# chanchanchan97/ICAFusion

Measured on NVIDIA H100. Metric: 640x512 RGB+IR pairs/sec end-to-end, higher is better.
Workload: dtype f16

## Files before the change

icafusion_b200/csrc/conv_common.cuh:

```cuda
#pragma once
#include "icaf_internal.cuh"

namespace icaf {

constexpr int BM = 128;
constexpr int BK = 64;
constexpr int kLag = 2;
constexpr int kThreads = 288;

enum AMode { A_GATHER = 0, A_TMA2D = 1, A_TMA4D = 2 };

struct ConvProblem {
  const __half* x; const float* bias; const __half* res; __half* y;
  const float* alpha; const float* beta;
  long long x_ld, res_ld, y_ld;
  const float2* ln_stats;
  const float* ln_s;
  float2* stats_out;
};
struct ConvParams {
  ConvProblem p[2];
  int M, N, K, k_pad;
  int B, Hi, Wi, Cin, Ho, Wo, kh, kw, stride, pad;
  int act, epi;
// ... 23 lines not shown
  r.y_ld = z ? P.p[1].y_ld : P.p[0].y_ld;
  r.ln_stats = z ? P.p[1].ln_stats : P.p[0].ln_stats; r.ln_s = z ? P.p[1].ln_s : P.p[0].ln_s;
  r.stats_out = z ? P.p[1].stats_out : P.p[0].stats_out;
  return r;
}

struct TileOrigin { int m0, tb, oy0, ox0; };
__device__ __forceinline__ void tile_origin(const ConvParams& P, int mtile, int& m0, int& tb, int& oy0, int& ox0) {
  m0 = mtile * BM; tb = 0; oy0 = 0; ox0 = 0;
  if (P.a_mode == A_TMA4D) {
    const int per_img = P.tiles_x * P.tiles_y;
    m0 = 0;
    tb = mtile / per_img;
    const int t = mtile - tb * per_img;
    oy0 = (t / P.tiles_x) * P.th;
    ox0 = (t % P.tiles_x) * P.tw;
  }
}

__device__ __forceinline__ void tile_row(const ConvParams& P, const TileOrigin& o, int row, int& m, bool& valid) {
  if (P.a_mode == A_TMA4D) {
    const int ry = row / P.tw, rx = row - ry * P.tw;
    m = (o.tb * P.Ho + o.oy0 + ry) * P.Wo + o.ox0 + rx;
    valid = ry < P.th && o.oy0 + ry < P.Ho;
  } else {
    m = o.m0 + row;
    valid = m < P.M;
  }
}

struct EpiRow {
  float ln_a, ln_mu;
  const float* ln_s;
  float sum, sumsq;
};
__device__ __forceinline__ void epi_row_ln(EpiRow& ex, const ConvParams& P, const ConvProblem& pr, int m, bool mvalid) {
  float su = 0.f, sq = 0.f;
  if (mvalid) {
    const float2* sp = pr.ln_stats + size_t(m) * P.ln_parts;
    for (int i = 0; i < P.ln_parts; ++i) { const float2 v = __ldg(sp + i); su += v.x; sq += v.y; }
  }
  const float mu = su * P.ln_inv_k;
  ex.ln_mu = mu;
  ex.ln_a = rsqrtf(fmaxf(sq * P.ln_inv_k - mu * mu, 0.f) + P.ln_eps);
}

struct StagedRow {
  int m;
  bool mvalid;
  float rbias;
  __half* yrow;
  const __half* rrow;
  EpiRow ex;
};
template <int BN, bool XM>
__device__ __forceinline__ void staged_row(StagedRow& r, const ConvParams& P, const ConvProblem& pr, const TileOrigin& o, int row, int n0) {
  tile_row(P, o, row, r.m, r.mvalid);
  r.rbias = ((P.epi & ICAF_EPI_BIAS_ROW) && pr.bias && r.mvalid) ? __ldg(pr.bias + r.m) : 0.f;
  r.yrow = pr.y + size_t(r.mvalid ? r.m : 0) * pr.y_ld;
  r.rrow = pr.res ? pr.res + size_t(r.mvalid ? r.m : 0) * pr.res_ld : nullptr;
  if (r.rrow && r.mvalid) {
    for (int cb = 0; cb < BN && n0 + cb < P.N; cb += 64) prefetch_l2(r.rrow + n0 + cb);
  }
  r.ex.sum = r.ex.sumsq = 0.f; r.ex.ln_a = 1.f; r.ex.ln_mu = 0.f; r.ex.ln_s = nullptr;
  if (XM) {
    r.ex.ln_s = pr.ln_s ? pr.ln_s + n0 : nullptr;
    if (P.ln_parts > 0) epi_row_ln(r.ex, P, pr, r.m, r.mvalid);
  }
}

__device__ __forceinline__ void epi_row_emit(const EpiRow& ex, const ConvParams& P, const ConvProblem& pr, int m, int n_begin, int n_end) {
  const int slots = (P.N + 31) >> 5;
  float2* sp = pr.stats_out + size_t(m) * slots;
  const int s0 = n_begin >> 5, s1 = min((n_end + 31) >> 5, slots);
  for (int i = s0; i < s1; ++i) sp[i] = i == s0 ? make_float2(ex.sum, ex.sumsq) : make_float2(0.f, 0.f);
}

template <int ACT, int RES>
__device__ __forceinline__ float epi_value(float a, float b, float rbias, float rf, float alpha, float beta) {
  float t = a + b + rbias;
  if (ACT == ICAF_ACT_SILU) t = silu_f(t);
  if (ACT == ICAF_ACT_GELU) t = gelu_erf_f(t);
  if (RES == 1) t = t + rf;
  if (RES == 2) t = alpha * rf + beta * t;
  return t;
}

template <int ACT, int RES, int XM = 0>
__device__ __forceinline__ void epi_chunk(const uint32_t (&acc)[32], const float* __restrict__ sb, float rbias,
                                          float alpha, float beta, const __half* __restrict__ rp,
                                          __half* __restrict__ yp, bool vec, int ncols, EpiRow& ex, int cb, bool do_store = true) {
  auto f = [&](int j, float rf) {
    float a = __uint_as_float(acc[j]);
    if (XM == 1) a = ex.ln_a * (a - ex.ln_mu * __ldg(ex.ln_s + cb + j));
    return epi_value<ACT, RES>(a, sb[j], rbias, rf, alpha, beta);
  };
  if (vec) {
#pragma unroll
    for (int q = 0; q < 4; ++q) {
      float rf[8];
      if (RES != 0) {
        uint4 rr = *reinterpret_cast<const uint4*>(rp + q * 8);
        const __half2* rh = reinterpret_cast<const __half2*>(&rr);
#pragma unroll
        for (int e = 0; e < 4; ++e) {
          const float2 r2 = __half22float2(rh[e]);
          rf[2 * e] = r2.x; rf[2 * e + 1] = r2.y;
        }
      } else {
#pragma unroll
        for (int e = 0; e < 8; ++e) rf[e] = 0.f;
      }
      float v[8];
#pragma unroll
      for (int e = 0; e < 8; ++e) v[e] = f(q * 8 + e, rf[e]);
      uint4 o;
      o.x = pack_half2(v[0], v[1]); o.y = pack_half2(v[2], v[3]);
      o.z = pack_half2(v[4], v[5]); o.w = pack_half2(v[6], v[7]);
      if (XM == 2) {
        const __half2* oh = reinterpret_cast<const __half2*>(&o);
#pragma unroll
        for (int e = 0; e < 4; ++e) {
          const float2 w = __half22float2(oh[e]);
          ex.sum += w.x + w.y;
          ex.sumsq += w.x * w.x + w.y * w.y;
        }
      }
      if (do_store) *reinterpret_cast<uint4*>(yp + q * 8) = o;
    }
  } else {
#pragma unroll
    for (int j = 0; j < 32; ++j) {
      if (j < ncols) {
        const float t = f(j, RES != 0 ? __half2float(rp[j]) : 0.f);
        const __half h = __float2half_rn(t);
        if (XM == 2) { const float w = __half2float(h); ex.sum += w; ex.sumsq += w * w; }
        yp[j] = h;
      }
    }
  }
}

__device__ __forceinline__ void load_staged(uint32_t (&acc)[32], const float* p) {
#pragma unroll
  for (int q = 0; q < 8; ++q) {
    const float4 v = *reinterpret_cast<const float4*>(p + 4 * q);
    acc[4 * q] = __float_as_uint(v.x); acc[4 * q + 1] = __float_as_uint(v.y);
    acc[4 * q + 2] = __float_as_uint(v.z); acc[4 * q + 3] = __float_as_uint(v.w);
  }
}

template <bool XM>
__device__ __forceinline__ void epi_dispatch(int mode_act, const uint32_t (&acc)[32], const float* sb, float rbias, float alpha,
                                             float beta, const __half* rp, __half* yp, bool vec, int ncols, EpiRow& ex, int cb) {
  if (XM) {
    switch (mode_act) {
      case 9: epi_chunk<0, 0, 1>(acc, sb, rbias, alpha, beta, rp, yp, vec, ncols, ex, cb); break;
      case 10: epi_chunk<2, 0, 1>(acc, sb, rbias, alpha, beta, rp, yp, vec, ncols, ex, cb); break;
      default: epi_chunk<0, 2, 2>(acc, sb, rbias, alpha, beta, rp, yp, vec, ncols, ex, cb); break;
    }
  } else {
    switch (mode_act) {
      case 0: epi_chunk<0, 0>(acc, sb, rbias, alpha, beta, rp, yp, vec, ncols, ex, cb); break;
      case 1: epi_chunk<0, 1>(acc, sb, rbias, alpha, beta, rp, yp, vec, ncols, ex, cb); break;
      case 2: epi_chunk<0, 2>(acc, sb, rbias, alpha, beta, rp, yp, vec, ncols, ex, cb); break;
      case 3: epi_chunk<1, 0>(acc, sb, rbias, alpha, beta, rp, yp, vec, ncols, ex, cb); break;
      case 4: epi_chunk<1, 1>(acc, sb, rbias, alpha, beta, rp, yp, vec, ncols, ex, cb); break;
      case 5: epi_chunk<1, 2>(acc, sb, rbias, alpha, beta, rp, yp, vec, ncols, ex, cb); break;
      case 6: epi_chunk<2, 0>(acc, sb, rbias, alpha, beta, rp, yp, vec, ncols, ex, cb); break;
      case 7: epi_chunk<2, 1>(acc, sb, rbias, alpha, beta, rp, yp, vec, ncols, ex, cb); break;
      default: epi_chunk<2, 2>(acc, sb, rbias, alpha, beta, rp, yp, vec, ncols, ex, cb); break;
    }
  }
}

template <bool XM>
__device__ __forceinline__ int epi_mode_act(const ConvParams& P, bool has_res) {
  if (XM) return P.ln_parts > 0 ? (P.act == ICAF_ACT_GELU ? 10 : 9) : 11;
  return P.act * 3 + ((P.epi & ICAF_EPI_SCALED_RES) ? 2 : (has_res ? 1 : 0));
}

template <bool XM>
__device__ __forceinline__ void epi_staged_chunk(int mode_act, const uint32_t (&acc)[32], StagedRow& r, const float* sbias,
                                                 float alpha, float beta, int cb, int nb, int N) {
  const int ncols = min(32, N - nb);
  const bool vec = ncols == 32 && ((reinterpret_cast<uintptr_t>(r.yrow + nb) & 15) == 0) &&
                   (!r.rrow || (reinterpret_cast<uintptr_t>(r.rrow + nb) & 15) == 0);
  epi_dispatch<XM>(mode_act, acc, sbias + cb, r.rbias, alpha, beta, r.rrow ? r.rrow + nb : nullptr, r.yrow + nb, vec, ncols,
                   r.ex, cb);
}

constexpr int kOutHalfBytes = BM * 64 * 2;

template <int PP, int NA>
__device__ __forceinline__ void take_cols16(const float (&acc0)[NA], const float (&acc1)[NA], float (&v)[16]) {
  constexpr int Q = PP < NA / 8 ? PP : NA / 8 - 1;
#pragma unroll
  for (int e = 0; e < 8; ++e) { v[e] = acc0[8 * Q + e]; v[8 + e] = acc1[8 * Q + e]; }
}

template <int ACT, int RES>
__device__ __forceinline__ void epi_fragments(const float (&v)[16], uint32_t sa, const float* sb, const float (&rb)[4],
                                              float alpha, float beta) {
#pragma unroll
  for (int h = 0; h < 2; ++h) {
    uint32_t r[4];
    if (RES != 0) ldmatrix_x4(r, sa + 8192u * h);
#pragma unroll
    for (int k = 0; k < 4; ++k) {
      const float2 b = *reinterpret_cast<const float2*>(sb + 8 * (k >> 1));
      const float rbias = rb[2 * h + (k & 1)];
      float2 rf = make_float2(0.f, 0.f);
      if (RES != 0) rf = __half22float2(*reinterpret_cast<const __half2*>(&r[k]));
      r[k] = pack_half2(epi_value<ACT, RES>(v[8 * h + 2 * k], b.x, rbias, rf.x, alpha, beta),
                        epi_value<ACT, RES>(v[8 * h + 2 * k + 1], b.y, rbias, rf.y, alpha, beta));
    }
    stmatrix_x4(sa + 8192u * h, r);
  }
}

__device__ __forceinline__ void epi_fragments_dispatch(int mode_act, const float (&v)[16], uint32_t sa, const float* sb,
                                                       const float (&rb)[4], float alpha, float beta) {
  switch (mode_act) {
    case 0: epi_fragments<0, 0>(v, sa, sb, rb, alpha, beta); break;
    case 1: epi_fragments<0, 1>(v, sa, sb, rb, alpha, beta); break;
    case 2: epi_fragments<0, 2>(v, sa, sb, rb, alpha, beta); break;
    case 3: epi_fragments<1, 0>(v, sa, sb, rb, alpha, beta); break;
    case 4: epi_fragments<1, 1>(v, sa, sb, rb, alpha, beta); break;
    case 5: epi_fragments<1, 2>(v, sa, sb, rb, alpha, beta); break;
    case 6: epi_fragments<2, 0>(v, sa, sb, rb, alpha, beta); break;
    case 7: epi_fragments<2, 1>(v, sa, sb, rb, alpha, beta); break;
    default: epi_fragments<2, 2>(v, sa, sb, rb, alpha, beta); break;
  }
}

template <int NA>
__device__ __forceinline__ void epi_tile_fragments(int mode_act, const float (&acc0)[NA], const float (&acc1)[NA], uint32_t sout,
                                                   const float* sbias, const float (&rb)[4], float alpha, float beta, int w, int l) {
  const uint32_t sa = sout + uint32_t(16 * w + (l & 7) + 8 * ((l >> 3) & 1)) * 128u;
  const float* sb = sbias + 2 * (l & 3);
#pragma unroll 1
  for (int p = 0; p < NA / 8; ++p) {
    float v[16];
    switch (p) {
      case 0: take_cols16<0>(acc0, acc1, v); break;
      case 1: take_cols16<1>(acc0, acc1, v); break;
      case 2: take_cols16<2>(acc0, acc1, v); break;
      case 3: take_cols16<3>(acc0, acc1, v); break;
      case 4: take_cols16<4>(acc0, acc1, v); break;
      case 5: take_cols16<5>(acc0, acc1, v); break;
      case 6: take_cols16<6>(acc0, acc1, v); break;
      default: take_cols16<7>(acc0, acc1, v); break;
    }
    const uint32_t a = sa + uint32_t(p >> 2) * uint32_t(kOutHalfBytes) + (uint32_t((2 * (p & 3) + (l >> 4)) ^ (l & 7)) << 4);
    epi_fragments_dispatch(mode_act, v, a, sb + 16 * p, rb, alpha, beta);
  }
}

__device__ __forceinline__ void fragment_row_bias(float (&rb)[4], const ConvParams& P, const ConvProblem& pr, const TileOrigin& o,
                                                  int w, int l) {
  if ((P.epi & ICAF_EPI_BIAS_ROW) && pr.bias) {
#pragma unroll
    for (int q = 0; q < 4; ++q) {
      int mq;
      bool vq;
      tile_row(P, o, 16 * w + (l >> 2) + 8 * (q & 1) + 64 * (q >> 1), mq, vq);
      rb[q] = vq ? __ldg(pr.bias + mq) : 0.f;
    }
  }
}

template <int BN>
__device__ __forceinline__ void tma_store_tile(const ConvParams& P, const CUtensorMap* map, uint32_t s, int n0, const TileOrigin& o) {
  const int halves = (BN == 128 && n0 + 64 < P.N) ? 2 : 1;
  for (int hh = 0; hh < halves; ++hh) {
    const uint32_t src = s + uint32_t(hh * kOutHalfBytes);
    if (P.a_mode == A_TMA4D) tma_store_4d(map, src, n0 + 64 * hh, o.ox0, o.oy0, o.tb);
    else tma_store_2d(map, src, n0 + 64 * hh, o.m0);
  }
  bulk_commit_group();
}

template <int BN>
__device__ __forceinline__ void tma_load_tile(const ConvParams& P, const CUtensorMap* map, uint32_t s, uint32_t bar, int n0,
                                              const TileOrigin& o) {
  const int halves = (BN == 128 && n0 + 64 < P.N) ? 2 : 1;
  const uint32_t half_bytes = P.a_mode == A_TMA4D ? uint32_t(P.tw * P.th) * 128u : uint32_t(kOutHalfBytes);
  mbar_arrive_expect_tx(bar, uint32_t(halves) * half_bytes);
  for (int hh = 0; hh < halves; ++hh) {
    const uint32_t dst = s + uint32_t(hh * kOutHalfBytes);
    if (P.a_mode == A_TMA4D) tma_load_4d(dst, map, bar, n0 + 64 * hh, o.ox0, o.oy0, o.tb);
    else tma_load_2d(dst, map, bar, n0 + 64 * hh, o.m0);
  }
}

struct ConvPlan {
  int kernel;
  int bn;
  unsigned grid_x, grid_y, grid_z, cluster;
  int smem;
  int tiles, m_tiles, n_tiles;
  int sms;
  bool persist;
  bool xm;
  int ctas;
};

}
```

icafusion_b200/csrc/conv_gemm.cu:

```cuda
#include <cstdlib>
#include <cstring>

#include "conv_common.cuh"

namespace icaf {

constexpr int kMaxStages = 10;
template <int BN>
struct SmemLayout {
  static constexpr int kABytes = BM * BK * 2;
  static constexpr int kBBytes = BN * BK * 2;
  static constexpr int kStageBytes = kABytes + kBBytes;
  static constexpr int kPitch = BN + 4;
  static constexpr int kAccBytes = BM * kPitch * 4;
  static constexpr int kTailBytes = 256 + BN * 4 + 1024;
  __host__ __device__ static int region(int stages) { return stages * kStageBytes > kAccBytes ? stages * kStageBytes : kAccBytes; }
  static int total(int stages) { return region(stages) + kTailBytes; }
};


template <int BN, bool kTmaA>
__device__ __forceinline__ void load_stage(const ConvParams& P, int a_mode, uint32_t sa, uint32_t bar, uint32_t bytes,
                                           const CUtensorMap* mw, const CUtensorMap* ma, int kb, int n0, const TileOrigin& o) {
  mbar_arrive_expect_tx(bar, bytes);
// ... 229 lines not shown
      *reinterpret_cast<float2*>(sacc + size_t(r) * L::kPitch + col) = make_float2(acc0[i], acc0[i + 1]);
      *reinterpret_cast<float2*>(sacc + size_t(r + 64) * L::kPitch + col) = make_float2(acc1[i], acc1[i + 1]);
    }
    if (splits > 1) { cluster_arrive(); cluster_wait(); cluster_arrive(); cluster_wait(); } else { named_bar_sync(1, 256); }
  } else {
    if (elect_one()) {
      const CUtensorMap* mw = bz ? &maps.w[1] : &maps.w[0];
      const CUtensorMap* ma = bz ? &maps.a[1] : &maps.a[0];
      const uint32_t a_bytes = a_mode == A_TMA2D ? L::kABytes : (a_mode == A_TMA4D ? uint32_t(P.tw * P.th) * 128u : 0u);
      const uint32_t bytes = L::kBBytes + a_bytes;
      int s = 0;
      uint32_t ph = 0;
      for (int kb = 0; kb < nkb; ++kb) {
        mbar_wait_quiet(empty_bar(s), ph ^ 1);
        load_stage<BN, false>(P, a_mode, smem_base + s * L::kStageBytes, full_bar(s), bytes, mw, ma, kb_begin + kb, n0, o);
        if (++s == kStages) { s = 0; ph ^= 1; }
      }
      if (tma_epi && has_res) {
        mbar_wait_quiet(empty_bar(s), ph ^ 1);
        tma_load_tile<BN>(P, bz ? &maps.res[1] : &maps.res[0], smem_base + uint32_t(s) * L::kStageBytes, res_bar, n0, o);
      }
    }
    __syncwarp();
    if (splits > 1) { cluster_arrive(); cluster_wait(); cluster_arrive(); cluster_wait(); }
  }
}

constexpr int kPersistThreads = 384;
constexpr int kHaloSlots = 2;
struct PersistLayout {
  static constexpr int kStageBytes = SmemLayout<128>::kStageBytes;
  static constexpr int kFilterBytes = SmemLayout<128>::kBBytes;
  static constexpr int kOutBytes = 2 * kOutHalfBytes;
  static constexpr int kPitch = 32 + 4;
  static constexpr int kChunkBytes = BM * kPitch * 4;
  static_assert(kChunkBytes <= kOutBytes, "the XM staged chunk lives in the output tile");
  __host__ __device__ static int ring_bytes(int stages, int halo_bytes) {
    return halo_bytes ? stages * kFilterBytes + kHaloSlots * halo_bytes : stages * kStageBytes;
  }
  __host__ __device__ static int bar_off(int stages, int halo_bytes) { return ring_bytes(stages, halo_bytes) + 2 * kOutBytes; }
  static int total(int stages, int halo_bytes) { return bar_off(stages, halo_bytes) + 256 + 2 * 128 * 4 + 1024; }
};

template <class FullBar, class HaloFull, class HandBack, class HaloBack>
__device__ __forceinline__ void halo_mma_loop(float (&acc0)[64], float (&acc1)[64], const ConvParams& P, uint32_t smem_base,
                                              int kStages, int g0, int h0, const int (&lane_px)[2], int l, FullBar full_bar,
                                              HaloFull halo_full, HandBack hand_back, HaloBack halo_back, int& s_last, int& h_last) {
  const int ncb = P.Cin / BK, hw = P.tw + 2;
  const uint32_t halo_base = smem_base + uint32_t(kStages * PersistLayout::kFilterBytes);
  int s = g0 % kStages, h = h0 % kHaloSlots;
  uint32_t ph = uint32_t(g0 / kStages) & 1u, hph = uint32_t(h0 / kHaloSlots) & 1u;
  int s_prev = s, h_prev = h;
  uint32_t fa[3][4][4];
  for (int cb = 0; cb < ncb; ++cb) {
    mbar_wait_quiet(halo_full(h), hph);
    const uint32_t sh = halo_base + uint32_t(h * P.halo_bytes);
#pragma unroll 1
    for (int ky = 0; ky < 3; ++ky) {
#pragma unroll
      for (int kx = 0; kx < 3; ++kx) {
        const int tap = 3 * ky + kx;
        mbar_wait_quiet(full_bar(s), ph);
        const uint32_t sb = smem_base + uint32_t(s * PersistLayout::kFilterBytes);
#pragma unroll
        for (int hm = 0; hm < 2; ++hm) {
          const int f = (2 * kx + hm) % 3;
          const int r = lane_px[hm] + ky * hw + kx;
          const uint32_t a = sh + uint32_t(r) * 128u;
#pragma unroll
          for (int kc = 0; kc < 4; ++kc) ldmatrix_x4(fa[f][kc], a + (uint32_t((2 * kc + (l >> 4)) ^ (r & 7)) << 4));
          wgmma_fence();
#pragma unroll
          for (int kc = 0; kc < 4; ++kc) {
            const uint64_t bd = gmma_desc_sw128(sb + 32 * kc);
            if (hm == 0) wgmma_rs<0>(acc0, fa[f][kc], bd, (cb | tap | kc) != 0);
            else wgmma_rs<0>(acc1, fa[f][kc], bd, (cb | tap | kc) != 0);
          }
          wgmma_commit();
          wgmma_wait<2>();
          if (hm == 1 && (cb | tap) != 0) {
            hand_back(s_prev);
            if (tap == 0) halo_back(h_prev);
          }
        }
        s_prev = s;
        if (++s == kStages) { s = 0; ph ^= 1; }
      }
    }
    h_prev = h;
    if (++h == kHaloSlots) { h = 0; hph ^= 1; }
  }
  s_last = s_prev;
  h_last = h_prev;
}

struct PersistTile { int z, n0; TileOrigin o; };
__device__ __forceinline__ PersistTile persist_tile(const ConvParams& P, int t) {
  PersistTile pt;
  const int r = t / P.n_tiles;
  const int mtile = r % P.m_tiles;
  pt.n0 = (t - r * P.n_tiles) * 128;
  pt.z = r / P.m_tiles;
  tile_origin(P, mtile, pt.o.m0, pt.o.tb, pt.o.oy0, pt.o.ox0);
  return pt;
}

template <int CC>
__device__ __forceinline__ void stage_chunk(const float (&acc0)[64], const float (&acc1)[64], float* sacc, int w, int l) {
#pragma unroll
  for (int i = 16 * CC; i < 16 * CC + 16; i += 2) {
    const int r = 16 * w + (l >> 2) + 8 * ((i >> 1) & 1), col = 8 * (i >> 2) - 32 * CC + 2 * (l & 3);
    *reinterpret_cast<float2*>(sacc + r * PersistLayout::kPitch + col) = make_float2(acc0[i], acc0[i + 1]);
    *reinterpret_cast<float2*>(sacc + (r + 64) * PersistLayout::kPitch + col) = make_float2(acc1[i], acc1[i + 1]);
  }
}

template <bool XM>
__global__ void __launch_bounds__(kPersistThreads, 1)
conv_gemm_persist_kernel(const ConvParams P, const __grid_constant__ ConvMaps maps) {
  extern __shared__ uint8_t smem_raw[];
  const uint32_t smem_base = (smem_u32(smem_raw) + 1023u) & ~1023u;
  using L = SmemLayout<128>;
  using PL = PersistLayout;
  const int kStages = P.stages;
  const bool halo = !XM && P.halo_bytes != 0;
  const uint32_t ring_bytes = uint32_t(PL::ring_bytes(kStages, P.halo_bytes));
  const uint32_t bar_off = uint32_t(PL::bar_off(kStages, P.halo_bytes));
  const uint32_t bar_base = smem_base + bar_off;
  auto full_bar = [&](int s) { return bar_base + 8u * s; };
  auto empty_bar = [&](int s) { return bar_base + 8u * (kMaxStages + s); };
  auto order_bar = [&](int c) { return bar_base + 8u * (2 * kMaxStages + c); };
  auto res_bar = [&](int c) { return bar_base + 8u * (2 * kMaxStages + 2 + c); };
  auto halo_full = [&](int h) { return bar_base + 8u * (2 * kMaxStages + 4 + h); };
  auto halo_empty = [&](int h) { return bar_base + 8u * (2 * kMaxStages + 4 + kHaloSlots + h); };
  static_assert(8 * (2 * kMaxStages + 4 + 2 * kHaloSlots) <= 256, "barriers");
  uint8_t* smem_gen = smem_raw + (smem_base - smem_u32(smem_raw));

  pdl_launch_dependents();
  const int tid = threadIdx.x;
  const int wg = tid >> 7;
  const int ncb = P.Cin / BK;
  const int nkb = halo ? 9 * ncb : P.k_pad / BK;
  const int a_mode = P.a_mode;
  const bool has_res = (P.epi & (ICAF_EPI_ADD_RES | ICAF_EPI_SCALED_RES)) != 0;
  if (tid == 0) {
    for (int s = 0; s < kStages; ++s) {
      mbar_init(full_bar(s), 1);
      mbar_init(empty_bar(s), 4);
    }
    mbar_init(order_bar(0), 4);
    mbar_init(order_bar(1), 4);
    mbar_init(res_bar(0), 1);
    mbar_init(res_bar(1), 1);
    for (int h = 0; h < kHaloSlots; ++h) {
      mbar_init(halo_full(h), 1);
      mbar_init(halo_empty(h), 4);
    }
    fence_mbar_init();
  }
  if (tid == 32) {
    tma_prefetch_desc(&maps.w[0]);
    tma_prefetch_desc(&maps.a[0]);
    if (P.tiles > P.m_tiles * P.n_tiles) { tma_prefetch_desc(&maps.w[1]); tma_prefetch_desc(&maps.a[1]); }
    if (!XM) {
      tma_prefetch_desc(&maps.y[0]);
      if (has_res) tma_prefetch_desc(&maps.res[0]);
    }
  }
  __syncthreads();
  pdl_wait();

  if (wg == 0) {
    setmaxnreg_dec<40>();
    if (tid < 32 && elect_one()) {
      const uint32_t a_bytes = a_mode == A_TMA2D ? L::kABytes : uint32_t(P.tw * P.th) * 128u;
      const uint32_t bytes = L::kBBytes + a_bytes;
      int s = 0, h = 0;
      uint32_t ph = 0, hph = 0;
      for (int tile = blockIdx.x; tile < P.tiles; tile += gridDim.x) {
        const PersistTile pt = persist_tile(P, tile);
        const CUtensorMap* mw = pt.z ? &maps.w[1] : &maps.w[0];
        const CUtensorMap* ma = pt.z ? &maps.a[1] : &maps.a[0];
        if (halo) {
          const uint32_t halo_tx = uint32_t((P.tw + 2) * (P.th + 2)) * 128u;
          for (int cb = 0; cb < ncb; ++cb) {
            mbar_wait_quiet(halo_empty(h), hph ^ 1);
            mbar_arrive_expect_tx(halo_full(h), halo_tx);
            tma_load_4d(smem_base + uint32_t(kStages * PL::kFilterBytes + h * P.halo_bytes), ma, halo_full(h), cb * BK,
                        pt.o.ox0 - 1, pt.o.oy0 - 1, pt.o.tb);
            if (++h == kHaloSlots) { h = 0; hph ^= 1; }
            for (int tap = 0; tap < 9; ++tap) {
              mbar_wait_quiet(empty_bar(s), ph ^ 1);
              mbar_arrive_expect_tx(full_bar(s), PL::kFilterBytes);
              tma_load_2d(smem_base + uint32_t(s * PL::kFilterBytes), mw, full_bar(s), tap * P.Cin + cb * BK, pt.n0);
              if (++s == kStages) { s = 0; ph ^= 1; }
            }
          }
          continue;
        }
        for (int kb = 0; kb < nkb; ++kb) {
          mbar_wait_quiet(empty_bar(s), ph ^ 1);
          load_stage<128, true>(P, a_mode, smem_base + s * L::kStageBytes, full_bar(s), bytes, mw, ma, kb, pt.n0, pt.o);
          if (++s == kStages) { s = 0; ph ^= 1; }
        }
      }
    }
    return;
  }

  setmaxnreg_inc<232>();
  const int c = wg - 1;
  const int t = tid & 127, w = t >> 5, l = t & 31;
  const int bar_id = 2 + c;
  const uint32_t sout = smem_base + ring_bytes + uint32_t(c * PL::kOutBytes);
  float* sacc = reinterpret_cast<float*>(smem_gen + ring_bytes + c * PL::kOutBytes);
  float* sbias = reinterpret_cast<float*>(smem_gen + bar_off + 256 + c * 128 * 4);
  int lane_px[2];
#pragma unroll
  for (int hm = 0; hm < 2; ++hm) {
    int m = 64 * hm + 16 * w + (l & 7) + 8 * ((l >> 3) & 1);
    if (m > P.tw * P.th - 1) m = P.tw * P.th - 1;
    const int py = P.tw ? m / P.tw : 0;
    lane_px[hm] = py * (P.tw + 2) + m - py * P.tw;
  }
  for (int tile = blockIdx.x + c * gridDim.x; tile < P.tiles; tile += 2 * gridDim.x) {
    const int j = (tile - int(blockIdx.x)) / int(gridDim.x);
    const PersistTile pt = persist_tile(P, tile);
    const ConvProblem pr = pick_problem(P, pt.z);
    const int n0 = pt.n0;
    const TileOrigin& o = pt.o;
    const float bias_r = (pr.bias && !(P.epi & ICAF_EPI_BIAS_ROW) && n0 + t < P.N) ? __ldg(pr.bias + n0 + t) : 0.f;
    float alpha = 0.f, beta = 1.f;
    if (P.epi & ICAF_EPI_SCALED_RES) { alpha = __ldg(pr.alpha); beta = __ldg(pr.beta); }
    StagedRow sr;
    float rb[4] = {0.f, 0.f, 0.f, 0.f};
    if (XM) {
      staged_row<128, XM>(sr, P, pr, o, t, n0);
    } else {
      fragment_row_bias(rb, P, pr, o, w, l);
      if (t == 0) {
        bulk_wait_group_read<0>();
        if (has_res) tma_load_tile<128>(P, pt.z ? &maps.res[1] : &maps.res[0], sout, res_bar(c), n0, o);
      }
      sbias[t] = bias_r;
      named_bar_sync(bar_id, 128);
    }

    float acc0[64], acc1[64];
#pragma unroll
    for (int i = 0; i < 64; ++i) { acc0[i] = 0.f; acc1[i] = 0.f; }
    auto hand_back = [&](int s) { if (l == 0) mbar_arrive(empty_bar(s)); };
    auto halo_back = [&](int h) { if (l == 0) mbar_arrive(halo_empty(h)); };
    const int g0 = j * nkb;
    if (j > 0) mbar_wait_quiet(order_bar(c), uint32_t((j >> 1) - (1 - c)) & 1u);
    int s_last, h_last = 0;
    if (halo) {
      halo_mma_loop(acc0, acc1, P, smem_base, kStages, g0, j * ncb, lane_px, l, full_bar, halo_full, hand_back, halo_back,
                    s_last, h_last);
    } else {
      s_last = mma_loop<128>(acc0, acc1, smem_base, kStages, nkb, g0 % kStages, uint32_t(g0 / kStages) & 1u, full_bar,
                             hand_back);
    }
    if (l == 0) mbar_arrive(order_bar(c ^ 1));
    wgmma_wait<0>();
    hand_back(s_last);
    if (halo) halo_back(h_last);

    if constexpr (!XM) {
      if (has_res) mbar_wait_quiet(res_bar(c), uint32_t(j >> 1) & 1u);
      epi_tile_fragments<64>(epi_mode_act<false>(P, has_res), acc0, acc1, sout, sbias, rb, alpha, beta, w, l);
      fence_proxy_async_smem();
      named_bar_sync(bar_id, 128);
      if (t == 0) {
        tma_store_tile<128>(P, pt.z ? &maps.y[1] : &maps.y[0], sout, n0, o);
        if (tile + 2 * int(gridDim.x) >= P.tiles) bulk_wait_group<0>();
      }
      continue;
    }

    const int mode_act = epi_mode_act<XM>(P, has_res);
    const float* arow = sacc + size_t(t) * PL::kPitch;
#pragma unroll 1
    for (int cc = 0; cc < 4; ++cc) {
      named_bar_sync(bar_id, 128);
      if (cc == 0) sbias[t] = bias_r;
      switch (cc) {
        case 0: stage_chunk<0>(acc0, acc1, sacc, w, l); break;
        case 1: stage_chunk<1>(acc0, acc1, sacc, w, l); break;
        case 2: stage_chunk<2>(acc0, acc1, sacc, w, l); break;
        default: stage_chunk<3>(acc0, acc1, sacc, w, l); break;
      }
      named_bar_sync(bar_id, 128);
      const int cb = 32 * cc;
      if (sr.mvalid && n0 + cb < P.N) {
        uint32_t acc[32];
        load_staged(acc, arow);
        epi_staged_chunk<XM>(mode_act, acc, sr, sbias, alpha, beta, cb, n0 + cb, P.N);
      }
    }
    if (mode_act == 11 && sr.mvalid && n0 < P.N) epi_row_emit(sr.ex, P, pr, sr.m, n0, min(n0 + 128, P.N));
  }
}

struct SimtParams { ConvParams P; const __half* w[2]; };
__global__ void conv_gemm_simt_kernel(const SimtParams S) {
  pdl_launch_dependents();
  pdl_wait();
  const ConvParams& P = S.P;
  const ConvProblem pr = pick_problem(P, blockIdx.z);
  const __half* w = blockIdx.z ? S.w[1] : S.w[0];
  long long idx = blockIdx.x * (long long)blockDim.x + threadIdx.x;
  if (idx >= (long long)P.M * P.N) return;
  int n = int(idx % P.N);
  int m = int(idx / P.N);
  int ox = m % P.Wo, t = m / P.Wo, oy = t % P.Ho, b = t / P.Ho;
  float acc = 0.f;
  for (int ky = 0; ky < P.kh; ++ky)
    for (int kx = 0; kx < P.kw; ++kx) {
      int iy = oy * P.stride - P.pad + ky, ix = ox * P.stride - P.pad + kx;
      if ((unsigned)iy >= (unsigned)P.Hi || (unsigned)ix >= (unsigned)P.Wi) continue;
      const __half* xp = pr.x + (size_t(b) * P.Hi * P.Wi + size_t(iy) * P.Wi + ix) * pr.x_ld;
      const __half* wp = w + size_t(n) * P.k_pad + (ky * P.kw + kx) * P.Cin;
      for (int c = 0; c < P.Cin; ++c) acc += __half2float(xp[c]) * __half2float(wp[c]);
    }
  if (pr.bias) acc += (P.epi & ICAF_EPI_BIAS_ROW) ? pr.bias[m] : pr.bias[n];
  if (P.act == ICAF_ACT_SILU) acc = acc / (1.0f + expf(-acc));
  else if (P.act == ICAF_ACT_GELU) acc = gelu_erf_f(acc);
  if (pr.res) {
    float rf = __half2float(pr.res[size_t(m) * pr.res_ld + n]);
    acc = (P.epi & ICAF_EPI_SCALED_RES) ? (*pr.alpha) * rf + (*pr.beta) * acc : acc + rf;
  }
  pr.y[size_t(m) * pr.y_ld + n] = __float2half_rn(acc);
}

static int fill_geom(const icaf_conv_geom* g, int n_io, ConvParams& P) {
  if (!g || n_io < 1 || n_io > 2) return set_error(ICAF_ERR_BAD_ARG, "conv2d: need 1 or 2 problems");
  if (!(g->Cin == 4 || g->Cin % 8 == 0)) return set_error(ICAF_ERR_UNSUPPORTED, "conv2d: Cin must be 4 or a multiple of 8");
  if (g->Cin == 4 && (g->Wi % 2 || g->stride % 2 || g->pad % 2 || g->kw % 2))
    return set_error(ICAF_ERR_UNSUPPORTED, "conv2d: packed-image (Cin=4) path needs even Wi, stride, pad, kw");
  if (g->k_pad % 64 || g->k_pad < g->kh * g->kw * g->Cin) return set_error(ICAF_ERR_BAD_ARG, "conv2d: bad k_pad");
  if (g->w_rows < g->Cout) return set_error(ICAF_ERR_BAD_ARG, "conv2d: w_rows < Cout");
  long long M = (long long)g->B * g->Ho * g->Wo;
  if (M <= 0 || M > 0x7fffffffLL || (long long)g->B * g->Hi * g->Wi > 0x7fffffffLL)
    return set_error(ICAF_ERR_BAD_ARG, "conv2d: size out of range");
  if ((g->epi & (ICAF_EPI_ADD_RES | ICAF_EPI_SCALED_RES)) == (ICAF_EPI_ADD_RES | ICAF_EPI_SCALED_RES))
    return set_error(ICAF_ERR_BAD_ARG, "conv2d: ADD_RES and SCALED_RES are exclusive");
  if ((g->epi & ICAF_EPI_LN_FOLD) && ((g->epi & ~ICAF_EPI_LN_FOLD) != 0 || !(g->act == ICAF_ACT_NONE || g->act == ICAF_ACT_GELU) ||
                                      g->kh != 1 || g->kw != 1 || g->stride != 1 || g->pad != 0))
    return set_error(ICAF_ERR_UNSUPPORTED, "conv2d: LN_FOLD is a linear-layer (1x1) epilogue without residual, activation none / GELU");
  if ((g->epi & ICAF_EPI_EMIT_STATS) && ((g->epi & ~ICAF_EPI_EMIT_STATS) != ICAF_EPI_SCALED_RES || g->act != ICAF_ACT_NONE))
    return set_error(ICAF_ERR_UNSUPPORTED, "conv2d: EMIT_STATS rides on the SCALED_RES epilogue without activation");
  P.M = int(M); P.N = g->Cout; P.K = g->kh * g->kw * g->Cin; P.k_pad = g->k_pad;
  P.B = g->B; P.Hi = g->Hi; P.Wi = g->Wi; P.Cin = g->Cin; P.Ho = g->Ho; P.Wo = g->Wo;
  P.kh = g->kh; P.kw = g->kw; P.stride = g->stride; P.pad = g->pad; P.act = g->act; P.epi = g->epi;
  P.a_mode = A_GATHER; P.tw = P.th = P.tiles_x = P.tiles_y = 0; P.stages = 2; P.splits = 1; P.cblk = 64;
  P.ln_parts = 0; P.ln_eps = 0.f; P.ln_inv_k = 0.f;
  P.m_tiles = P.n_tiles = P.tiles = 0;
  P.tma_epi = 0;
  P.halo_bytes = 0;
  memset(P.p, 0, sizeof(P.p));
  return ICAF_OK;
}

static int fill_params(const icaf_conv_geom* g, const icaf_conv_io* io, int n_io, ConvParams& P, const __half* (&w)[2]) {
  if (!io) return set_error(ICAF_ERR_BAD_ARG, "conv2d: null io");
  if (int rc = fill_geom(g, n_io, P)) return rc;
  for (int i = 0; i < 2; ++i) {
    const icaf_conv_io& s = io[i < n_io ? i : 0];
    bool need_res = g->epi & (ICAF_EPI_ADD_RES | ICAF_EPI_SCALED_RES);
    if (!s.x || !s.w || !s.y || (need_res && !s.res) || ((g->epi & ICAF_EPI_SCALED_RES) && (!s.alpha || !s.beta)))
      return set_error(ICAF_ERR_BAD_ARG, "conv2d: null pointer");
    if ((reinterpret_cast<uintptr_t>(s.x) & 15) || (reinterpret_cast<uintptr_t>(s.w) & 15) || (s.x_ld % 8 && g->Cin != 4) ||
        (g->Cin == 4 && s.x_ld != 4))
      return set_error(ICAF_ERR_BAD_ARG, "conv2d: x / w must be 16-byte aligned with x_ld a multiple of 8");
    if ((g->epi & ICAF_EPI_LN_FOLD) && (!s.ln_stats || !s.ln_colsum || s.ln_parts < 1 || s.ln_parts > 64))
      return set_error(ICAF_ERR_BAD_ARG, "conv2d: LN_FOLD needs ln_stats, ln_colsum and 1..64 partials per row");
    if ((g->epi & ICAF_EPI_EMIT_STATS) && !s.stats_out) return set_error(ICAF_ERR_BAD_ARG, "conv2d: EMIT_STATS needs stats_out");
    if (i > 0 && (g->epi & ICAF_EPI_LN_FOLD) && (s.ln_parts != io[0].ln_parts || s.ln_eps != io[0].ln_eps))
      return set_error(ICAF_ERR_BAD_ARG, "conv2d: grouped problems must share ln_parts / ln_eps");
    P.p[i] = ConvProblem{(const __half*)s.x, s.bias, need_res ? (const __half*)s.res : nullptr, (__half*)s.y, s.alpha, s.beta,
                         s.x_ld, s.res_ld, s.y_ld,
                         (g->epi & ICAF_EPI_LN_FOLD) ? (const float2*)s.ln_stats : nullptr,
                         (g->epi & ICAF_EPI_LN_FOLD) ? s.ln_colsum : nullptr,
                         (g->epi & ICAF_EPI_EMIT_STATS) ? (float2*)s.stats_out : nullptr};
    if (i == 0 && (g->epi & ICAF_EPI_LN_FOLD)) { P.ln_parts = s.ln_parts; P.ln_eps = s.ln_eps; P.ln_inv_k = 1.0f / float(P.K); }
    w[i] = (const __half*)s.w;
  }
  return ICAF_OK;
}

static void plan_a_mode(const icaf_conv_geom* g, ConvParams& P) {
  if (g->kh == 1 && g->kw == 1 && g->stride == 1 && g->pad == 0 && g->Cin % 8 == 0) {
    P.a_mode = A_TMA2D;
    return;
  }
  if (g->Cin % 64 == 0 && g->stride <= 2) {
    int best_tw = 0, best_th = 0;
    double best_u = 0.0;
    for (int tw = 1; tw <= 128 && tw <= g->Wo; ++tw) {
      if (g->Wo % tw || tw * g->stride > 256) continue;
      int th = 128 / tw;
      if (th > g->Ho) th = g->Ho;
      if (th * g->stride > 256) th = 256 / g->stride;
      int ty = (g->Ho + th - 1) / th;
      double u = double(g->Wo) * g->Ho / (double(g->Wo / tw) * ty * 128.0);
      if (u > best_u + 1e-9 || (u > best_u - 1e-9 && tw > best_tw)) { best_u = u; best_tw = tw; best_th = th; }
    }
    if (best_u >= 0.6) {
      P.a_mode = A_TMA4D; P.tw = best_tw; P.th = best_th; P.tiles_x = g->Wo / best_tw; P.tiles_y = (g->Ho + best_th - 1) / best_th;
    }
  }
}

template <int BN>
static int plan_tc(ConvParams& P, int n_io, ConvPlan& pl) {
  using L = SmemLayout<BN>;
  constexpr int kSmemCap = 227 * 1024;
  const int mt = P.a_mode == A_TMA4D ? P.B * P.tiles_x * P.tiles_y : (P.M + BM - 1) / BM;
  if (P.a_mode == A_TMA4D && !(P.tw >= 1 && P.th >= 1 && P.tw * P.th <= BM && P.tiles_x * P.tw >= P.Wo && P.tiles_y * P.th >= P.Ho &&
                               P.cblk == 64 && P.Cin % 64 == 0))
    return set_error(ICAF_ERR_BAD_ARG, "conv2d(tc): 4-D tiles must cover the map with at most 128 pixels each, 64-channel blocks");
  unsigned gx = unsigned(mt), gy = unsigned((P.N + BN - 1) / BN), gz = unsigned(n_io);
  const long long tiles = (long long)gx * gy * gz;
  const int budget = (tiles <= pl.sms || BN > 64) ? kSmemCap : (kSmemCap / 2 - 1024);
  int stages = (budget - L::kTailBytes) / L::kStageBytes;
  const int nkb = P.k_pad / BK;
  if (stages > nkb) stages = nkb;
  if (stages > kMaxStages) stages = kMaxStages;
  if (stages < 2) stages = 2;
  int splits = 1;
  if (tiles * 2 <= pl.sms && nkb >= 8) {
    splits = int(pl.sms / tiles);
    if (splits > 8) splits = 8;
    if (splits > nkb / 4) splits = nkb / 4;
    if (splits < 1) splits = 1;
  }
  if (splits > 1) {
    const int per = (nkb + splits - 1) / splits;
    if (stages > per) stages = per < 2 ? 2 : per;
    gx *= splits;
  }
  if (stages > kMaxStages || L::total(stages) > kSmemCap)
    return set_error(ICAF_ERR_BAD_ARG, "conv2d(tc): shared-memory plan exceeds the ring / 227 KB");
  P.stages = stages;
  P.splits = splits;
  pl.kernel = ICAF_KERNEL_TC; pl.bn = BN;
  pl.grid_x = gx; pl.grid_y = gy; pl.grid_z = gz; pl.cluster = unsigned(splits);
  pl.smem = L::total(stages);
  pl.tiles = int(tiles); pl.m_tiles = mt; pl.n_tiles = int(gy);
  pl.persist = false; pl.ctas = int(gx * gy * gz);
  return ICAF_OK;
}

static int plan_persist(ConvParams& P, ConvPlan& pl) {
  constexpr int kSmemCap = 227 * 1024;
  const bool halo = !pl.xm && P.a_mode == A_TMA4D && P.kh == 3 && P.kw == 3 && P.stride == 1 && P.pad == 1;
  P.halo_bytes = halo ? ((P.tw + 2) * (P.th + 2) * 128 + 1023) / 1024 * 1024 : 0;
  int stages = kMaxStages;
  while (stages > 2 && PersistLayout::total(stages, P.halo_bytes) > kSmemCap) --stages;
  if (PersistLayout::total(stages, P.halo_bytes) > kSmemCap)
    return set_error(ICAF_ERR_BAD_ARG, "conv2d(persist): shared-memory plan exceeds 227 KB");
  P.stages = stages;
  P.m_tiles = pl.m_tiles; P.n_tiles = pl.n_tiles; P.tiles = pl.tiles;
  pl.persist = true;
  pl.ctas = pl.tiles < pl.sms ? pl.tiles : pl.sms;
  pl.smem = PersistLayout::total(stages, P.halo_bytes);
  return ICAF_OK;
}

template <int BN>
static int encode_maps(const ConvParams& P, const __half* const (&w)[2], const icaf_conv_geom* g, int n_io, bool out_maps,
                       ConvMaps& maps) {
  memset(&maps, 0, sizeof(maps));
  for (int i = 0; i < n_io; ++i) {
    int rc = encode_tmap_2d(&maps.w[i], w[i], (uint64_t)P.k_pad, (uint64_t)g->w_rows, (uint64_t)P.k_pad * 2, BK, BN);
    if (rc) return rc;
    const ConvProblem& pr = P.p[i];
    if (P.a_mode == A_TMA2D)
      rc = encode_tmap_2d(&maps.a[i], pr.x, (uint64_t)P.Cin, (uint64_t)P.M, (uint64_t)pr.x_ld * 2, BK, BM);
    else if (P.a_mode == A_TMA4D && P.halo_bytes)
      rc = encode_tmap_nhwc(&maps.a[i], pr.x, P.Cin, P.Wi, P.Hi, P.B, pr.x_ld, BK, P.tw + 2, P.th + 2, 1, 1);
    else if (P.a_mode == A_TMA4D)
      rc = encode_tmap_nhwc(&maps.a[i], pr.x, P.Cin, P.Wi, P.Hi, P.B, pr.x_ld, BK, P.tw * P.stride, P.th * P.stride, P.stride,
                            P.stride);
    if (rc) return rc;
    if (out_maps) {
      auto out_map = [&](CUtensorMap* m, const __half* base, long long ld) {
        return P.a_mode != A_TMA4D ? encode_tmap_2d(m, base, (uint64_t)P.N, (uint64_t)P.M, (uint64_t)ld * 2, 64, BM)
                                   : encode_tmap_nhwc(m, base, P.N, P.Wo, P.Ho, P.B, ld, 64, P.tw, P.th, 1, 1);
      };
      if ((rc = out_map(&maps.y[i], pr.y, pr.y_ld))) return rc;
      if (pr.res && (rc = out_map(&maps.res[i], pr.res, pr.res_ld))) return rc;
    }
  }
  if (n_io == 1) { maps.w[1] = maps.w[0]; maps.a[1] = maps.a[0]; maps.y[1] = maps.y[0]; maps.res[1] = maps.res[0]; }
  return ICAF_OK;
}

template <int BN>
static int launch_conv(const ConvParams& P, const ConvPlan& pl, const __half* const (&w)[2], const icaf_conv_geom* g, int n_io,
                       cudaStream_t st) {
  void (*kernel)(ConvParams, ConvMaps) = pl.xm ? conv_gemm_tc_kernel<BN, true> : conv_gemm_tc_kernel<BN, false>;
  if (pl.persist) kernel = pl.xm ? conv_gemm_persist_kernel<true> : conv_gemm_persist_kernel<false>;
  static bool configured[2][2][kMaxDevices] = {};
  if (int rc = configure_smem(kernel, 227 * 1024, configured[pl.persist][pl.xm], "conv2d: cudaFuncSetAttribute")) return rc;
  ConvMaps maps;
  if (int rc = encode_maps<BN>(P, w, g, n_io, P.tma_epi != 0, maps)) return rc;
  const dim3 grid = pl.persist ? dim3(unsigned(pl.ctas)) : dim3(pl.grid_x, pl.grid_y, pl.grid_z);
  return launch_kc("conv2d_fwd", kernel, grid, dim3(pl.persist ? kPersistThreads : kThreads), (size_t)pl.smem, st, pl.cluster, P, maps);
}

static int plan_conv(const icaf_conv_geom* g, int n_io, int sms, bool tma_out, ConvParams& P, ConvPlan& pl) {
  memset(&pl, 0, sizeof(pl));
  pl.sms = sms;
  if (sms < 1) return set_error(ICAF_ERR_BAD_ARG, "conv2d: SM count must be positive");
  pl.xm = (P.epi & (ICAF_EPI_LN_FOLD | ICAF_EPI_EMIT_STATS)) != 0;
  plan_a_mode(g, P);
  const long long mt = P.a_mode == A_TMA4D ? (long long)P.B * P.tiles_x * P.tiles_y : (P.M + BM - 1) / BM;
  auto ctas = [&](int bn) { return mt * ((P.N + bn - 1) / bn) * n_io; };
  int bn = 32;
  if (P.N > 64 && ctas(128) >= sms) bn = 128;
  else if (P.N > 32 && ctas(64) >= sms) bn = 64;
  int rc;
  switch (bn) {
    case 128:
      rc = plan_tc<128>(P, n_io, pl);
      if (!rc && (pl.xm || tma_out) && P.a_mode != A_GATHER && P.splits == 1 && pl.tiles > sms) rc = plan_persist(P, pl);
      break;
    case 64: rc = plan_tc<64>(P, n_io, pl); break;
    default: rc = plan_tc<32>(P, n_io, pl); break;
  }
  if (rc) return rc;
  P.tma_epi = !pl.xm && (pl.persist || (tma_out && P.splits == 1 && pl.bn >= 64)) ? 1 : 0;
  return ICAF_OK;
}

}

using namespace icaf;


extern "C" int icaf_conv2d_plan(const icaf_conv_geom* g, int n_io, int sm_count, int pair_mode, icaf_conv_plan* out) {
  if (!out) return set_error(ICAF_ERR_BAD_ARG, "conv2d_plan: null output");
  ConvParams P;
  int rc = fill_geom(g, n_io, P);
  if (rc) return rc;
  ConvPlan pl;
  (void)pair_mode;
  rc = plan_conv(g, n_io, sm_count, true, P, pl);
  if (rc) return rc;
  out->kernel = pl.kernel; out->bn = pl.bn; out->a_mode = P.a_mode;
  out->tile_w = P.tw; out->tile_h = P.th; out->tiles_x = P.tiles_x; out->tiles_y = P.tiles_y;
  out->cblk = P.cblk; out->halo = 0; out->stages = P.stages; out->splits = P.splits;
  out->grid_x = int(pl.grid_x); out->grid_y = int(pl.grid_y); out->grid_z = int(pl.grid_z); out->cluster = int(pl.cluster);
  out->smem_bytes = pl.smem; out->work_items = pl.tiles; out->ctas = pl.ctas;
  return ICAF_OK;
}

extern "C" int icaf_conv2d_fwd(const icaf_conv_geom* g, const icaf_conv_io* io, int n_io, void* stream) {
  ConvParams P;
  const __half* w[2];
  int rc = fill_params(g, io, n_io, P, w);
  if (rc) return rc;
  bool tma_out = true;
  for (int i = 0; i < n_io; ++i) {
    const ConvProblem& pr = P.p[i];
    tma_out = tma_out && (reinterpret_cast<uintptr_t>(pr.y) & 15) == 0 && pr.y_ld % 8 == 0 &&
              (!pr.res || ((reinterpret_cast<uintptr_t>(pr.res) & 15) == 0 && pr.res_ld % 8 == 0));
  }
  ConvPlan pl;
  rc = plan_conv(g, n_io, sm_count_cached(), tma_out, P, pl);
  if (rc) return rc;
  cudaStream_t st = (cudaStream_t)stream;
  switch (pl.bn) {
    case 128: return launch_conv<128>(P, pl, w, g, n_io, st);
    case 64: return launch_conv<64>(P, pl, w, g, n_io, st);
    case 32: return launch_conv<32>(P, pl, w, g, n_io, st);
    default: return set_error(ICAF_ERR_BAD_ARG, "conv2d: the planner produced an unknown tile width");
  }
}

extern "C" int icaf_conv2d_fwd_simt(const icaf_conv_geom* g, const icaf_conv_io* io, int n_io, void* stream) {
  SimtParams S;
  int rc = fill_params(g, io, n_io, S.P, S.w);
  if (rc) return rc;
  long long total = (long long)S.P.M * S.P.N;
  dim3 grid(blocks_for(total, 256), 1, n_io);
  return launch_k("conv2d_fwd_simt", conv_gemm_simt_kernel, dim3(grid), dim3(256), 0, (cudaStream_t)stream, S);
}
```

Before: 2134.

## Add specialized halo-tiled stem conv kernel for 3x3 Cin=16 layers

Adds a dedicated kernel for 3x3 stride-1 convolutions with 16 input channels. It loads an input halo tile into shared memory once via cp.async and reuses it across all nine taps with register-sourced wgmma, instead of gathering an im2col A tile for every K block. The filter stays resident through TMA and the output goes out by TMA store. This cuts redundant gather traffic on the early high-resolution layers, at the cost of a narrowly gated extra code path with its own swizzle and halo-indexing logic.

```diff
diff --git a/icafusion_b200/csrc/conv_common.cuh b/icafusion_b200/csrc/conv_common.cuh
--- a/icafusion_b200/csrc/conv_common.cuh
+++ b/icafusion_b200/csrc/conv_common.cuh
@@ -349,6 +349,7 @@
   int tiles, m_tiles, n_tiles;
   int sms;
   bool persist;
+  bool stem;
   bool xm;
   int ctas;
 };
diff --git a/icafusion_b200/csrc/conv_gemm.cu b/icafusion_b200/csrc/conv_gemm.cu
--- a/icafusion_b200/csrc/conv_gemm.cu
+++ b/icafusion_b200/csrc/conv_gemm.cu
@@ -555,6 +555,130 @@
   }
 }
 
+constexpr int kStemThreads = 128;
+struct StemLayout {
+  static constexpr int kFilterBytes = 3 * SmemLayout<64>::kBBytes;
+  static constexpr int kBiasOff = kFilterBytes;
+  static constexpr int kBarOff = kBiasOff + 64 * 4;
+  static constexpr int kHaloOff = kFilterBytes + 1024;
+  __host__ __device__ static int pitch(int Wo) { return (Wo < BM ? Wo : BM) + 2; }
+  __host__ __device__ static int runs(int Wo) { return 1 + (BM - 1 + Wo - 1) / Wo; }
+  static int total(int Wo) {
+    const int halo = runs(Wo) * 3 * pitch(Wo) * 32;
+    return kHaloOff + (halo > kOutHalfBytes ? halo : kOutHalfBytes) + 1024;
+  }
+};
+
+__global__ void __launch_bounds__(kStemThreads, 4)
+conv_stem_kernel(const ConvParams P, const __grid_constant__ ConvMaps maps) {
+  extern __shared__ uint8_t smem_raw[];
+  using SL = StemLayout;
+  const uint32_t smem_base = (smem_u32(smem_raw) + 1023u) & ~1023u;
+  uint8_t* smem_gen = smem_raw + (smem_base - smem_u32(smem_raw));
+  const uint32_t bar = smem_base + SL::kBarOff;
+  const uint32_t halo = smem_base + SL::kHaloOff;
+  float* sbias = reinterpret_cast<float*>(smem_gen + SL::kBiasOff);
+
+  pdl_launch_dependents();
+  const int t = threadIdx.x, w = t >> 5, l = t & 31;
+  const int bz = blockIdx.z, n0 = blockIdx.y * 64;
+  const ConvProblem pr = pick_problem(P, bz);
+  const TileOrigin o{int(blockIdx.x) * BM, 0, 0, 0};
+  const int g0 = o.m0 / P.Wo, ox0 = o.m0 - g0 * P.Wo;
+  const int len0 = min(P.Wo - ox0, BM);
+  const int nruns = 1 + (BM - len0 + P.Wo - 1) / P.Wo;
+  const int pitch = SL::pitch(P.Wo);
+  int lane_hp[2];
+#pragma unroll
+  for (int hm = 0; hm < 2; ++hm) {
+    const int r = 64 * hm + 16 * w + (l & 7) + 8 * ((l >> 3) & 1);
+    int j = 0, p = r;
+    if (r >= len0) {
+      const int q = (r - len0) / P.Wo;
+      j = 1 + q;
+      p = r - len0 - q * P.Wo;
+    }
+    lane_hp[hm] = 3 * j * pitch + p;
+  }
+  if (t == 0) {
+    mbar_init(bar, 1);
+    fence_mbar_init();
+  }
+  if (t == 32) {
+    tma_prefetch_desc(bz ? &maps.w[1] : &maps.w[0]);
+    tma_prefetch_desc(bz ? &maps.y[1] : &maps.y[0]);
+  }
+  __syncthreads();
+  pdl_wait();
+
+  if (t == 0) {
+    const CUtensorMap* mw = bz ? &maps.w[1] : &maps.w[0];
+    mbar_arrive_expect_tx(bar, SL::kFilterBytes);
+#pragma unroll 1
+    for (int kb = 0; kb < 3; ++kb) tma_load_2d(smem_base + uint32_t(kb * SmemLayout<64>::kBBytes), mw, bar, kb * BK, n0);
+  }
+  if (t < 64) sbias[t] = (pr.bias && !(P.epi & ICAF_EPI_BIAS_ROW) && n0 + t < P.N) ? __ldg(pr.bias + n0 + t) : 0.f;
+  float rb[4] = {0.f, 0.f, 0.f, 0.f};
+  fragment_row_bias(rb, P, pr, o, w, l);
+
+  const int c = t & 1;
+#pragma unroll 1
+  for (int j = 0; j < nruns; ++j) {
+    const int g = g0 + j;
+    const int xs = j ? 0 : ox0;
+    const int len = j ? min(P.Wo, BM - len0 - (j - 1) * P.Wo) : len0;
+    const int b = g / P.Ho, oy = g - b * P.Ho;
+    const bool gv = g < P.B * P.Ho;
+#pragma unroll
+    for (int ty = 0; ty < 3; ++ty) {
+      const int iy = oy + ty - 1;
+      const bool rv = gv && (unsigned)iy < (unsigned)P.Hi;
+      const __half* src = pr.x + (rv ? (size_t(b) * P.Hi + iy) * P.Wi * pr.x_ld : 0) + 8 * c;
+      const int h0 = (3 * j + ty) * pitch;
+      for (int px = t >> 1; px < len + 2; px += kStemThreads / 2) {
+        const int ix = xs - 1 + px, h = h0 + px;
+        const bool ok = rv && (unsigned)ix < (unsigned)P.Wi;
+        cp_async16(halo + uint32_t(h) * 32u + (uint32_t(c ^ ((h >> 2) & 1)) << 4), ok ? src + size_t(ix) * pr.x_ld : pr.x, ok);
+      }
+    }
+  }
+  cp_async_commit();
+  cp_async_wait<0>();
+  __syncthreads();
+  mbar_wait_quiet(bar, 0);
+
+  float acc0[32], acc1[32];
+#pragma unroll
+  for (int i = 0; i < 32; ++i) { acc0[i] = 0.f; acc1[i] = 0.f; }
+  uint32_t fa[3][2][4];
+#pragma unroll
+  for (int tap = 0; tap < 9; ++tap) {
+    const int f = tap % 3;
+    const int off = (tap / 3) * pitch + tap % 3;
+#pragma unroll
+    for (int hm = 0; hm < 2; ++hm) {
+      const int h = lane_hp[hm] + off;
+      ldmatrix_x4(fa[f][hm], halo + uint32_t(h) * 32u + (uint32_t((l >> 4) ^ ((h >> 2) & 1)) << 4));
+    }
+    wgmma_fence();
+    const uint64_t bd = gmma_desc_sw128(smem_base + uint32_t((tap >> 2) * SmemLayout<64>::kBBytes + 32 * (tap & 3)));
+    wgmma_rs<0>(acc0, fa[f][0], bd, tap != 0);
+    wgmma_rs<0>(acc1, fa[f][1], bd, tap != 0);
+    wgmma_commit();
+    wgmma_wait<2>();
+  }
+  wgmma_wait<0>();
+  __syncthreads();
+
+  epi_tile_fragments<32>(epi_mode_act<false>(P, false), acc0, acc1, halo, sbias, rb, 0.f, 1.f, w, l);
+  fence_proxy_async_smem();
+  __syncthreads();
+  if (t == 0) {
+    tma_store_tile<64>(P, bz ? &maps.y[1] : &maps.y[0], halo, n0, o);
+    bulk_wait_group<0>();
+  }
+}
+
 struct SimtParams { ConvParams P; const __half* w[2]; };
 __global__ void conv_gemm_simt_kernel(const SimtParams S) {
   pdl_launch_dependents();
@@ -755,12 +879,15 @@
                        cudaStream_t st) {
   void (*kernel)(ConvParams, ConvMaps) = pl.xm ? conv_gemm_tc_kernel<BN, true> : conv_gemm_tc_kernel<BN, false>;
   if (pl.persist) kernel = pl.xm ? conv_gemm_persist_kernel<true> : conv_gemm_persist_kernel<false>;
-  static bool configured[2][2][kMaxDevices] = {};
-  if (int rc = configure_smem(kernel, 227 * 1024, configured[pl.persist][pl.xm], "conv2d: cudaFuncSetAttribute")) return rc;
+  if (pl.stem) kernel = conv_stem_kernel;
+  static bool configured[3][2][kMaxDevices] = {};
+  const int family = pl.stem ? 2 : (pl.persist ? 1 : 0);
+  if (int rc = configure_smem(kernel, 227 * 1024, configured[family][pl.xm], "conv2d: cudaFuncSetAttribute")) return rc;
   ConvMaps maps;
   if (int rc = encode_maps<BN>(P, w, g, n_io, P.tma_epi != 0, maps)) return rc;
   const dim3 grid = pl.persist ? dim3(unsigned(pl.ctas)) : dim3(pl.grid_x, pl.grid_y, pl.grid_z);
-  return launch_kc("conv2d_fwd", kernel, grid, dim3(pl.persist ? kPersistThreads : kThreads), (size_t)pl.smem, st, pl.cluster, P, maps);
+  const int threads = pl.persist ? kPersistThreads : (pl.stem ? kStemThreads : kThreads);
+  return launch_kc("conv2d_fwd", kernel, grid, dim3(threads), (size_t)pl.smem, st, pl.cluster, P, maps);
 }
 
 static int plan_conv(const icaf_conv_geom* g, int n_io, int sms, bool tma_out, ConvParams& P, ConvPlan& pl) {
@@ -780,7 +907,15 @@
       rc = plan_tc<128>(P, n_io, pl);
       if (!rc && (pl.xm || tma_out) && P.a_mode != A_GATHER && P.splits == 1 && pl.tiles > sms) rc = plan_persist(P, pl);
       break;
-    case 64: rc = plan_tc<64>(P, n_io, pl); break;
+    case 64:
+      rc = plan_tc<64>(P, n_io, pl);
+      if (!rc && !pl.xm && tma_out && P.a_mode == A_GATHER && P.splits == 1 && P.Cin == 16 && P.kh == 3 && P.kw == 3 &&
+          P.stride == 1 && P.pad == 1 && !(P.epi & (ICAF_EPI_ADD_RES | ICAF_EPI_SCALED_RES))) {
+        P.stages = 1;
+        pl.stem = true;
+        pl.smem = StemLayout::total(P.Wo);
+      }
+      break;
     default: rc = plan_tc<32>(P, n_io, pl); break;
   }
   if (rc) return rc;
```

New measurement: 2204, median of 6. 3.3% higher.
